# SLebailly/Ignis-MasterThesis

Hardware: AMD Instinct MI355X
Metric: Mrays/s (primary+secondary) at fixed spp; per-pixel L2 vs CPU ref (higher is better)
Workload: dtype f32; 1 GPU; diamond_scene.json 1000x1000, 256 spp = 32 iterations x spi 8, path tracer max_depth 64, seed 0; scene=diamond_scene.json, width=1000, height=1000, spp=256, spi=8, parallelism=single GPU

## Files before the change

ignis-masterthesis_amd/csrc/igx_device.hip:

```cpp
#include "igx.h"

#include "device_math.h"
#include "device_scene.h"
#include "igx_kernels.h"
#include "../host/bvh_build.h"
#include "../host/light_select.h"
#include "../host/lds_plan.h"
#include "../host/aov_plan.h"
#include "../host/film_tools.h"

#include <hip/hip_runtime.h>

#include <algorithm>
#include <array>
#include <chrono>
#include <map>
#include <cmath>
#include <cstring>
#include <condition_variable>
#include <deque>
#include <memory>
#include <mutex>
#include <string>
#include <thread>
#include <vector>
#include <type_traits>

using namespace igxd;

#ifndef IGX_PART
#define IGX_PART 0
#endif

namespace igxh {

constexpr int BLOCK = 256;
constexpr int BLOCK_WIDE = LDS_PLAN_BLOCK_WIDE;
static_assert(BLOCK == LDS_PLAN_BLOCK, "host/lds_plan.h plans for BLOCK-thread blocks");
[[maybe_unused]] constexpr int MAX_BLOCKS_PER_CU = 8;
[[maybe_unused]] constexpr int MAX_STACK = 128;
constexpr int MAX_BOUNCES = 256;
constexpr long long MAX_CHUNK_PATHS = 1ll << 27;
constexpr int SLOT_BITS = 27;
constexpr uint32_t SLOT_MASK = (1u << SLOT_BITS) - 1;
[[maybe_unused]] constexpr int MAX_ENCLOSING = 31;
static_assert(MAX_CHUNK_PATHS <= (1ll << SLOT_BITS), "path slots must fit the slot bits");
#ifndef EXTEND_WAVES
#define EXTEND_WAVES 4
#endif
#ifndef EXTEND_WAVES_FULL
#define EXTEND_WAVES_FULL 3
#endif
#ifndef EXTEND_WAVES_LDS
#define EXTEND_WAVES_LDS 4
#endif


constexpr int NSH = 64;
constexpr int CSTRIDE = 16;
constexpr int CROW = NSH * CSTRIDE;
// ... 589 lines not shown
            if (st.cls)
                for (int k = 0; k < 16; ++k)
                    if (st.cls[20 + k]) atomicAdd(&stats[54 + k], st.cls[20 + k]);
        }
    }
}

template <class CountOf>
__device__ __forceinline__ int take_group(int* work, int& s, uint64_t& done, int n, CountOf count_of, int claimed = -1) {
    unsigned long long* const done_mask = reinterpret_cast<unsigned long long*>(work + CROW);
    for (;;) {
        if (!((done >> s) & 1ull)) {
            int v = claimed;
            claimed = -1;
            if (v < 0) {
                v = 0;
                if (lane_id() == 0) v = atomicAdd(work + s * CSTRIDE, 1);
                v = __builtin_amdgcn_readfirstlane(v);
            }
            if (v * 64 < n) return v;
            if (lane_id() == 0 && !((__hip_atomic_load(done_mask, __ATOMIC_RELAXED, __HIP_MEMORY_SCOPE_AGENT) >> s) & 1ull))
                atomicOr(done_mask, 1ull << s);
            done |= 1ull << s;
        }
        unsigned long long m = 0;
        if (lane_id() == 0) m = __hip_atomic_load(done_mask, __ATOMIC_RELAXED, __HIP_MEMORY_SCOPE_AGENT);
        done |= (uint64_t)(uint32_t)__builtin_amdgcn_readfirstlane((int)(uint32_t)m) |
                ((uint64_t)(uint32_t)__builtin_amdgcn_readfirstlane((int)(uint32_t)(m >> 32)) << 32);
        const uint64_t open = ~done;
        if (!open) return -1;
        const int r = (s + 1) & (NSH - 1);
        const uint64_t rot = (open >> r) | (r ? (open << (NSH - r)) : 0ull);
        s = (r + __ffsll((unsigned long long)rot) - 1) & (NSH - 1);
        n = count_of(s);
    }
}

__device__ __forceinline__ PathState camera_path(const FrameArgs& fa, const SceneView& sv, int i) {
    const GenPath g = gen_path(fa, sv, i);
    PathState ps;
    ps.o = g.o;
    ps.d = g.d;
    ps.counter = g.counter;
    ps.seed = g.seed;
    ps.depth = g.depth;
    ps.slot = i;
    ps.contrib = mk(1, 1, 1);
    ps.inv_pdf = 0;
    ps.eta = 1.0f;
    ps.inside = -1;
    return ps;
}

template <int V0, bool STATS, bool LDS, int BT = BLOCK>
__global__ void __launch_bounds__(BT, LDS ? EXTEND_WAVES_LDS : (variant_full(V0) ? EXTEND_WAVES_FULL : EXTEND_WAVES)) k_extend(FrameArgs fa, SceneView gsv, PathBuf in, PathBuf out, ShadowBuf sh,
                                                  float4* L, KernelCounters kc, int tail_threshold) {
    static_assert(BT == BLOCK || (LDS && BT == BLOCK_WIDE), "the wide block is the LDS-staged kernel's");
    constexpr bool SHADE_LDS = BT > BLOCK;
    constexpr int V = LDS ? kernel_variant(V0, true) : (EXTEND_TREELET ? kernel_variant(V0, false) : V0);
    __shared__ int stack_mem[LDS_STACK * BT];
    extern __shared__ float4 lds_scene[];
    const TStack ts = make_tstack<BT>(stack_mem, LDS_STACK, gsv.spill);
    const bool gen = fa.gen_n > 0;
    if (!gen && row_total(kc.cnt_in) <= tail_threshold) return;
    const SceneView sv = LDS ? stage_scene_lds<BT, SHADE_LDS>(gsv, lds_scene) : stage_treelet<BT>(gsv, lds_scene);
    TraceStats st{0, 0, 0, 0, 0, 0, 0};
    __shared__ unsigned long long cls_mem[STATS ? BT / 64 * 36 : 1];
    if constexpr (STATS) {
        st.cls = cls_mem + 36 * (threadIdx.x >> 6);
        if (lane_id() < 36) st.cls[lane_id()] = 0;
    }
    const WaveWork w = wave_work<BT>();
    int s = w.s;
    auto count_of = [&](int sh_) {
        if (gen) {
            const int g = gen_shard_count(fa.gen_n, sh_);
            return ShardCount{g, g, g};
        }
        return shard_count(kc.cnt_in, sh_);
    };
    ShardCount sc = count_of(s);
    uint64_t done = 0;
    int p0 = w.k * 64;
    int claimed = -1;
    unsigned long long t_last = STATS ? __builtin_amdgcn_s_memtime() : 0;
    for (;;) {
        if (fa.dynamic) {
            const int g = take_group(kc.work, s, done, sc.n, [&](int sh_) {
                sc = count_of(sh_);
                return sc.n;
            }, claimed);
            if (g < 0) break;
            p0 = g * 64;
        } else if (p0 >= sc.n) {
            break;
        }
        if (STATS) phase_mark(st, t_last, 3);
        const int ns = sc.n;
        int* const c_out = kc.cnt_out + s * CSTRIDE;
        int* const c_sh = kc.cnt_shadow + s * CSTRIDE;
        const int q = p0 + lane_id();
        const int pos = (fa.reverse && !gen) ? ns - 1 - q : q;
        bool alive = false, has_shadow = false, has_l = false;
        PathState ps;
        ShadowRec sr;
        f3 Lacc = mk(0, 0, 0);
        ps.depth = 0;
        if (q < ns) {
            if (gen) {
                const int i = ((pos >> 6) << 12) | (s << 6) | (pos & 63);
                ps = camera_path(fa, sv, i);
                if (variant_full(V0) && IGX_AOV && fa.aov_di) fa.aov_di[i] = fa.aov_nee[i] = make_float4(0, 0, 0, 0);
            } else {
                ps = load_path(in, path_index(in, s, pos, sc));
            }
            if (!STATS && ps.depth > 0) alive = extend_step<STATS, V>(fa, sv, ts, ps, Lacc, has_l, has_shadow, sr, st);
// ... 794 lines not shown
[[maybe_unused]] constexpr size_t TREELET_FRONT = 1280;

inline long long row_total(const Slot& s, int row) {
    if (row == 0) return s.n0;
    long long t = 0;
    const int* r = s.pinned + (size_t)row * CROW;
    for (int k = 0; k < NSH; ++k) t += r[k * CSTRIDE] + r[k * CSTRIDE + 1] + r[k * CSTRIDE + 2];
    return t;
}

}

using namespace igxh;

struct igx_device {
    int hip_device = 0;
    hipStream_t stream = nullptr;
    hipStream_t stream2 = nullptr;
    hipStream_t tail_stream = nullptr;
    std::string last_error;
    int num_cus = 256;
    size_t mem_total = 0;
    bool timing = false;
    bool instrument = false;
    int64_t capacity_opt = 0;
    int64_t slot_budget_mb = 0;
    int stream_slots = 2;
    int concurrent_opt = 1;
    int concurrent_start_pct = 10;
    int tail_pairs_opt = -1;
    int64_t treelet_opt = -1;
    bool tree_dirty = true;
    int tree_ext = 0, tree_shadow = 0;
    int64_t tail_opt = -1;
    int64_t tail_last_opt = -1;
    bool fuse_generate = true;
    int split_opt = -1;
    int refill_opt = -1;
    int shadow_ifif_opt = -1;
    int64_t lds_scene_max = 48 * 1024;
    size_t lds_scene_bytes = 0;
    int lds_shading_opt = -1;
    int64_t lds_shading_max = 48 * 1024;
    size_t lds_shading_bytes = 0;
    int ext_block = BLOCK;
    size_t lds_shading_tab[LDS_TAB_COUNT] = {};
    size_t lds_per_block = 64 * 1024;
    size_t table_bytes = 0;
    size_t shading_bytes = 0;
    int leaf_size = 4;
    int classify_opt = 4;
    int shadow_classes_opt = 1;
    int shadow_optimistic_opt = -1;
    int dynamic_opt = DYN_EXTEND | DYN_REFILL_TRACE | DYN_REFILL_SHADOW;
    int group_order_opt = -1;
    int face_normals_opt = 1;
    int face_shade_opt = 1;
    float sah_node_cost = 1.0f;
    int bvh_bins = 32;
    int bvh_bins_tlas = 32;
    bool spatial_splits = false;
    bool rebuild_bvh = false;
    bool has_scene = false;
    std::vector<void*> scene_allocs;
    SceneView sv{};
    igx_camera cam_desc{};
    int variant = 0;
    int bvh_width = 2;
    bool quantized = false;
    int quantize_opt = -1;
    int nf4 = 4;
    int bvh_width_opt = 0;
    bool full_shading = false;
    bool full_shading_opt = false;
    bool enclosing_opt = true;
    int scene_depth = 0;
    int* spill_main = nullptr;
    int* spill_tail = nullptr;
    int* spill_shadow = nullptr;
    int* spill_main2 = nullptr;
    hipStream_t shadow_stream = nullptr;
    int overlap_shadow_opt = 1;
    Slot slots[2];
    int next_slot = 0;
    unsigned long long* dstats = nullptr;
    unsigned long long* tail_counts = nullptr;
    float* ray_list = nullptr;
    size_t ray_list_cap = 0;
    float* fb = nullptr;
    size_t fb_count = 0;
    bool aov_on = false;
    float* aov_fb[2] = {nullptr, nullptr};
    int fb_w = 0, fb_h = 0;
    uint64_t iteration_count = 0;
    int info_mode = INFO_OFF;
    bool info_follow_specular = false;
    int info_max_depth = 8;
    float* info_fb[AOV_INFO_COUNT] = {nullptr, nullptr, nullptr};
    uint64_t info_count[AOV_INFO_COUNT] = {0, 0, 0};
    std::vector<std::pair<hipEvent_t, hipEvent_t>> info_timed;
    void* post_buf[4] = {nullptr, nullptr, nullptr, nullptr};
    size_t post_cap[4] = {0, 0, 0, 0};
    igx_stats stats{};
    int async_opt = 1;
    struct AsyncRender* async = nullptr;
    int host_wait_us = 20;
// ... 18 lines not shown
#define HIPCHK(expr)                                                                                  \
    do {                                                                                              \
        hipError_t e_ = (expr);                                                                       \
        if (e_ != hipSuccess)                                                                         \
            return fail(dev, e_ == hipErrorOutOfMemory ? IGX_ERR_OUT_OF_MEMORY : IGX_ERR_HIP,         \
                        std::string(#expr) + ": " + hipGetErrorString(e_));                           \
    } while (0)

template <typename T>
igx_status upload(igx_device* dev, const std::vector<T>& v, const T** out) {
    size_t bytes = std::max<size_t>(v.size() * sizeof(T), 16);
    void* p = nullptr;
    HIPCHK(hipMalloc(&p, bytes));
    dev->scene_allocs.push_back(p);
    if (!v.empty()) HIPCHK(hipMemcpy(p, v.data(), v.size() * sizeof(T), hipMemcpyHostToDevice));
    *out = reinterpret_cast<const T*>(p);
    return IGX_OK;
}

void free_scene(igx_device* dev) {
    for (void* p : dev->scene_allocs) (void)hipFree(p);
    dev->scene_allocs.clear();
    dev->spill_main = dev->spill_tail = dev->spill_shadow = dev->spill_main2 = nullptr;
    dev->has_scene = false;
}

int max_grid(const igx_device* dev) {
    return std::max(GRID_QUANTUM, dev->num_cus * MAX_BLOCKS_PER_CU / GRID_QUANTUM * GRID_QUANTUM);
}

igx_status configure_stack(igx_device* dev) {
    const int need = dev->scene_depth;
    const int extra = std::max(0, need - LDS_STACK);
    dev->variant = (dev->bvh_width >= 4 ? 2 : 0) | (extra > 0 ? 1 : 0) | (dev->full_shading ? 4 : 0) | (dev->quantized ? VARIANT_Q4 : 0);
    const size_t threads = (size_t)max_grid(dev) * BLOCK;
    for (int k = 0; k < 4; ++k) {
        int*& old = k == 0 ? dev->spill_main : k == 1 ? dev->spill_tail : k == 2 ? dev->spill_shadow : dev->spill_main2;
        if (old) {
            auto it = std::find(dev->scene_allocs.begin(), dev->scene_allocs.end(), (void*)old);
            if (it != dev->scene_allocs.end()) dev->scene_allocs.erase(it);
            (void)hipFree(old);
            old = nullptr;
        }
        void* p = nullptr;
        HIPCHK(hipMalloc(&p, std::max<size_t>(16, (size_t)extra * threads * sizeof(int))));
        dev->scene_allocs.push_back(p);
        (k == 0 ? dev->spill_main : k == 1 ? dev->spill_tail : k == 2 ? dev->spill_shadow : dev->spill_main2) = static_cast<int*>(p);
    }
    dev->sv.spill = dev->spill_main;
    return IGX_OK;
}

void free_slot_buffers(Slot& s) {
    void* ptrs[] = {s.pa.p0, s.pa.p1, s.pa.p2, s.pa.p3, s.pb.p0, s.pb.p1, s.pb.p2, s.pb.p3, s.sh.s0, s.sh.s1, s.sh.s2, s.L, s.hb.h, s.hb.prim,
                    s.aov_di, s.aov_nee};
    for (void* p : ptrs)
        if (p) (void)hipFree(p);
    s.pa = PathBuf{};
    s.pb = PathBuf{};
    s.sh = ShadowBuf{};
    s.hb = HitBuf{};
    s.L = nullptr;
    s.aov_di = s.aov_nee = nullptr;
    s.cap = 0;
    s.shard_cap = 0;
}

igx_status ensure_slot(igx_device* dev, Slot& s, size_t cap, bool hits, bool region_c, bool aov) {
    if (!s.ctr) {
        HIPCHK(hipMalloc((void**)&s.ctr, CTR_INTS * sizeof(int)));
        HIPCHK(hipHostMalloc((void**)&s.pinned, CTR_INTS * sizeof(int), hipHostMallocDefault));
        HIPCHK(hipEventCreateWithFlags(&s.done, hipEventDisableTiming));
        std::memset(s.pinned, 0, CTR_INTS * sizeof(int));
    }
    if (s.cap >= cap && (!hits || s.hb.h) && (!region_c || s.pa.c_base) && (!aov || s.aov_di)) return IGX_OK;
    free_slot_buffers(s);
    const int shard_cap = (int)((cap + 64 * NSH - 1) / (64 * NSH)) * 64;
    const size_t recs = (size_t)shard_cap * NSH;
    auto alloc4 = [&](float4** p, size_t k) -> igx_status { HIPCHK(hipMalloc((void**)p, k * sizeof(float4))); return IGX_OK; };
    igx_status st;
    const size_t precs = region_c ? 2 * recs : recs;
    if ((st = alloc4(&s.pa.p0, precs)) || (st = alloc4(&s.pa.p1, precs)) || (st = alloc4(&s.pa.p2, precs))) return st;
    HIPCHK(hipMalloc((void**)&s.pa.p3, precs * sizeof(float2)));
    if ((st = alloc4(&s.pb.p0, precs)) || (st = alloc4(&s.pb.p1, precs)) || (st = alloc4(&s.pb.p2, precs))) return st;
    HIPCHK(hipMalloc((void**)&s.pb.p3, precs * sizeof(float2)));
    s.pa.c_base = s.pb.c_base = region_c ? (int)recs : 0;
    if ((st = alloc4(&s.sh.s0, recs)) || (st = alloc4(&s.sh.s1, recs)) || (st = alloc4(&s.sh.s2, recs))) return st;
    if ((st = alloc4(&s.L, cap))) return st;
    if (aov && ((st = alloc4(&s.aov_di, cap)) || (st = alloc4(&s.aov_nee, cap)))) return st;
    if (hits) {
        if ((st = alloc4(&s.hb.h, recs))) return st;
        HIPCHK(hipMalloc((void**)&s.hb.prim, recs * sizeof(int)));
    }
    s.pa.shard_cap = s.pb.shard_cap = s.sh.shard_cap = shard_cap;
    s.cap = cap;
    s.shard_cap = shard_cap;
    return IGX_OK;
}

hipEvent_t slot_event(Slot& s) {
    if (s.ev_next >= s.ev_pool.size()) {
        hipEvent_t e;
        (void)hipEventCreate(&e);
        s.ev_pool.push_back(e);
    }
    return s.ev_pool[s.ev_next++];
}

int grid_for(igx_device* dev, long long items, int blocks_per_cu, int block = BLOCK) {
    const long long q = NSH / (block / 64);
    long long need = (items + block - 1) / block;
    long long cap = (long long)dev->num_cus * std::min(blocks_per_cu, MAX_BLOCKS_PER_CU * BLOCK / block);
    long long g = std::min((need + q - 1) / q * q, std::max(q, cap / q * q));
    return (int)std::max(q, g);
}

#endif

constexpr size_t SPLIT_TABLE_BYTES = 64u << 20;
#ifndef GROUP_ORDER_AUTO
#define GROUP_ORDER_AUTO 0
#endif
inline bool use_tail_pairs(const igx_device* dev) {
    return dev->lds_scene_bytes == 0 && (dev->tail_pairs_opt < 0 ? true : dev->tail_pairs_opt != 0);
}
inline size_t tree_bytes(const igx_device* dev, int nodes) { return (size_t)nodes * dev->nf4 * 16; }
inline int refill_min(const igx_device* dev) { return dev->refill_opt >= 0 ? dev->refill_opt : 16; }
inline bool use_refill(const igx_device* dev) {
    return refill_min(dev) > 0 && (dev->lds_scene_bytes == 0 || dev->refill_opt > 0);
}
inline bool use_split(const igx_device* dev) {
    return dev->split_opt >= 0 ? dev->split_opt != 0 : (dev->lds_scene_bytes == 0 && dev->table_bytes > SPLIT_TABLE_BYTES);
}
inline bool use_shadow_ifif(const igx_device* dev) {
    return dev->shadow_ifif_opt >= 0 ? dev->shadow_ifif_opt != 0 : use_split(dev);
}
inline bool use_shadow_optimistic(const igx_device* dev, bool split, bool aovs) {
    if (dev->shadow_optimistic_opt == 0 || split || aovs) return false;
    return dev->shadow_optimistic_opt > 0 || (dev->shadow_classes_opt && dev->sv.num_enc > 0);
}
// ... 5 lines not shown
        case 1: MACRO(1); break;              \
        case 2: MACRO(2); break;              \
        case 3: MACRO(3); break;              \
        case 2 | VARIANT_Q4: MACRO(130); break; \
        default: MACRO(131); break;           \
        }                                     \
    } while (0)
#define IGX_DISPATCH_VARIANT8(v, MACRO)       \
    do {                                      \
        switch ((v) & (7 | VARIANT_Q4)) {     \
        case 0: MACRO(0); break;              \
        case 1: MACRO(1); break;              \
        case 2: MACRO(2); break;              \
        case 3: MACRO(3); break;              \
        case 4: MACRO(4); break;              \
        case 5: MACRO(5); break;              \
        case 6: MACRO(6); break;              \
        case 7: MACRO(7); break;              \
        case 2 | VARIANT_Q4: MACRO(130); break; \
        case 3 | VARIANT_Q4: MACRO(131); break; \
        case 6 | VARIANT_Q4: MACRO(134); break; \
        default: MACRO(135); break;           \
        }                                     \
    } while (0)

template <bool STATS>
void launch_extend_wide(igx_device* dev, Slot& s, int grid, const FrameArgs& fa, const PathBuf& in, const PathBuf& out,
                        const KernelCounters& kc, int tail) {
    const size_t dyn = lds_pad16(dev->lds_scene_bytes) + dev->lds_shading_bytes;
#define L_EXTW(S) hipLaunchKernelGGL((k_extend<S, STATS, true, BLOCK_WIDE>), dim3(grid), dim3(BLOCK_WIDE), dyn, dev->stream, fa, dev->sv, in, out, s.sh, s.L, kc, tail)
    IGX_DISPATCH_VARIANT8(dev->variant, L_EXTW);
#undef L_EXTW
}
template <typename K>
hipError_t raise_dynamic_lds(K kernel, size_t dyn) {
    static std::map<std::pair<const void*, int>, size_t> raised;
    int d = 0;
    (void)hipGetDevice(&d);
    const void* const fn = reinterpret_cast<const void*>(kernel);
    size_t& have = raised[{fn, d}];
    if (dyn <= have) return hipSuccess;
    const hipError_t e = hipFuncSetAttribute(fn, hipFuncAttributeMaxDynamicSharedMemorySize, (int)dyn);
    if (e == hipSuccess) have = dyn;
    return e;
}
template <bool STATS>
hipError_t extend_wide_prepare(int v, size_t dyn) {
#define L_PREP(S) return raise_dynamic_lds(k_extend<S, STATS, true, BLOCK_WIDE>, dyn)
    IGX_DISPATCH_VARIANT8(v, L_PREP);
#undef L_PREP
    return hipSuccess;
}

template <bool STATS>
void launch_extend(igx_device* dev, Slot& s, int grid, const FrameArgs& fa, const PathBuf& in, const PathBuf& out,
                   const KernelCounters& kc, int tail) {
    if (dev->ext_block == BLOCK_WIDE) {
        launch_extend_wide<STATS>(dev, s, grid, fa, in, out, kc, tail);
        return;
    }
    if (dev->lds_scene_bytes) {
#define L_EXTL(S) hipLaunchKernelGGL((k_extend<S, STATS, true>), dim3(grid), dim3(BLOCK), dev->lds_scene_bytes, dev->stream, fa, dev->sv, in, out, s.sh, s.L, kc, tail)
        IGX_DISPATCH_VARIANT8(dev->variant, L_EXTL);
#undef L_EXTL
        return;
    }
    SceneView tsv = dev->sv;
    tsv.tree_n = dev->tree_ext;
#define L_EXT(S) hipLaunchKernelGGL((k_extend<S, STATS, false>), dim3(grid), dim3(BLOCK), tree_bytes(dev, tsv.tree_n), dev->stream, fa, tsv, in, out, s.sh, s.L, kc, tail)
    IGX_DISPATCH_VARIANT8(dev->variant, L_EXT);
#undef L_EXT
}
template <bool STATS>
void launch_trace(igx_device* dev, Slot& s, int grid, const FrameArgs& fa, const PathBuf& in, const int* cnt, int tail,
                  int* work) {
    if (use_refill(dev)) {
#define L_TRR(S)                                                                                                        \
    if (dev->lds_scene_bytes)                                                                                            \
        hipLaunchKernelGGL((k_trace_refill<S, STATS, true>), dim3(grid), dim3(BLOCK), dev->lds_scene_bytes, dev->stream, fa, \
                           dev->sv, in, s.hb, cnt, tail, dev->dstats, refill_min(dev), work);                            \
    else                                                                                                                 \
        hipLaunchKernelGGL((k_trace_refill<S, STATS, false>), dim3(grid), dim3(BLOCK), 0, dev->stream, fa, dev->sv, in, s.hb, \
                           cnt, tail, dev->dstats, refill_min(dev), work)
        IGX_DISPATCH_VARIANT(dev->variant, L_TRR);
#undef L_TRR
        return;
    }
    if (dev->lds_scene_bytes) {
#define L_TRL(S) hipLaunchKernelGGL((k_trace<S, STATS, 1, true>), dim3(grid), dim3(BLOCK), dev->lds_scene_bytes, dev->stream, fa, dev->sv, in, s.hb, cnt, tail, dev->dstats)
        IGX_DISPATCH_VARIANT(dev->variant, L_TRL);
#undef L_TRL
        return;
    }
#define L_TR(S) hipLaunchKernelGGL((k_trace<S, STATS, 5, false>), dim3(grid), dim3(BLOCK), 0, dev->stream, fa, dev->sv, in, s.hb, cnt, tail, dev->dstats)
    IGX_DISPATCH_VARIANT(dev->variant, L_TR);
#undef L_TR
}
template <bool STATS>
void launch_shadow(igx_device* dev, Slot& s, int grid, const int* cnt, int* work, hipStream_t strm) {
    SceneView tsv = dev->sv;
    tsv.tree_n = dev->tree_shadow;
    if (strm != dev->stream) tsv.spill = dev->spill_shadow;
    if (use_refill(dev)) {
#define L_SHR(S)                                                                                                        \
    if (dev->lds_scene_bytes)                                                                                            \
        hipLaunchKernelGGL((k_shadow_refill<S, STATS, true>), dim3(grid), dim3(BLOCK), dev->lds_scene_bytes, strm,   \
                           tsv, s.sh, s.L, cnt, dev->dstats, refill_min(dev), work);                                 \
    else                                                                                                                 \
        hipLaunchKernelGGL((k_shadow_refill<S, STATS, false>), dim3(grid), dim3(BLOCK), tree_bytes(dev, tsv.tree_n), strm, \
// ... 233 lines not shown
    s.timed.clear();
    s.ev_next = 0;
    s.pending = false;
    return IGX_OK;
}

igx_status drain(igx_device* dev) {
    igx_status st;
    if ((st = ::wait_idle(dev)) || (st = harvest(dev, dev->slots[0])) || (st = harvest(dev, dev->slots[1]))) return st;
    HIPCHK(hipStreamSynchronize(dev->stream));
    HIPCHK(hipStreamSynchronize(dev->stream2));
    HIPCHK(hipStreamSynchronize(dev->shadow_stream));
    HIPCHK(hipStreamSynchronize(dev->tail_stream));
    for (auto& t : dev->info_timed) {
        float ms = 0;
        if (hipEventElapsedTime(&ms, t.first, t.second) == hipSuccess) dev->stats.ms_generate += ms;
        (void)hipEventDestroy(t.first);
        (void)hipEventDestroy(t.second);
    }
    dev->info_timed.clear();
    unsigned long long tc[2] = {0, 0};
    HIPCHK(hipMemcpy(tc, dev->tail_counts, sizeof(tc), hipMemcpyDeviceToHost));
    HIPCHK(hipMemset(dev->tail_counts, 0, sizeof(tc)));
    dev->stats.bounce_rays += tc[0];
    dev->stats.shadow_rays += tc[1];
    dev->stats.tail_bounce_rays += tc[0];
    dev->stats.tail_shadow_rays += tc[1];
    return IGX_OK;
}

#ifndef LDS_SHADING_AUTO
#define LDS_SHADING_AUTO 1
#endif
constexpr size_t EXTEND_FIXED_LDS = 2 * MAX_ENC_BOXES * sizeof(float4) + BLOCK_WIDE / 64 * 36 * sizeof(unsigned long long);
void configure_lds(igx_device* dev) {
    dev->lds_scene_bytes = dev->lds_shading_bytes = 0;
    dev->ext_block = BLOCK;
    if (!dev->has_scene) return;
    LdsPlanInput in;
    in.traversal_bytes = dev->table_bytes;
    in.traversal_max = dev->lds_scene_max;
    for (int k = 0; k < LDS_TAB_COUNT; ++k) in.shading_bytes[k] = dev->lds_shading_tab[k];
    in.shading_max = dev->lds_shading_max;
    in.shading_on = dev->lds_shading_opt < 0 ? LDS_SHADING_AUTO != 0 : dev->lds_shading_opt != 0;
    in.stack_bytes_per_thread = LDS_STACK * sizeof(int);
    in.fixed_bytes = EXTEND_FIXED_LDS;
    in.lds_per_block = dev->lds_per_block;
    LdsPlan p = plan_lds(in);
    if (p.block_threads == BLOCK_WIDE) {
        const size_t dyn = lds_pad16(p.traversal_bytes) + p.shading_bytes;
        (void)hipSetDevice(dev->hip_device);
        hipError_t e = extend_wide_prepare<false>(dev->variant, dyn);
        if (e == hipSuccess) e = extend_wide_prepare<true>(dev->variant, dyn);
        if (e != hipSuccess) {
            (void)hipGetLastError();
            dev->last_error = std::string("lds_shading: the wide k_extend's LDS block was refused (") + hipGetErrorString(e) +
                              "); keeping the 256-thread layout";
            p.block_threads = BLOCK;
            p.shading_bytes = 0;
        }
    }
    dev->lds_scene_bytes = p.traversal_bytes;
    dev->lds_shading_bytes = p.shading_bytes;
    dev->ext_block = p.block_threads;
}

void configure_treelet(igx_device* dev) {
    dev->tree_ext = dev->tree_shadow = 0;
    dev->tree_dirty = false;
    if (!dev->has_scene || dev->lds_scene_bytes || dev->treelet_opt == 0) return;
    int cap = (int)std::min<size_t>(TREELET_FRONT, (size_t)dev->sv.num_nodes);
    if (dev->treelet_opt > 0) cap = (int)std::min<int64_t>(cap, dev->treelet_opt);
    const int v = dev->variant;
    const bool refill = use_refill(dev);
    auto fit = [&](auto blocks) {
        const int nb0 = blocks((size_t)0);
        int lo = 0, hi = cap;
        while (lo < hi) {
            const int mid = (lo + hi + 1) / 2;
            if (blocks(tree_bytes(dev, mid)) >= nb0) lo = mid;
            else hi = mid - 1;
        }
        return lo;
    };
    if (EXTEND_TREELET) dev->tree_ext = fit([&](size_t t) { return extend_blocks_per_cu<false>(v, 0, t); });
    if (SHADOW_TREELET && !(refill && use_shadow_ifif(dev))) dev->tree_shadow = fit([&](size_t t) { return shadow_blocks_per_cu<false>(v, 0, refill, t); });
}

long long valid_pixels_in_chunk(const FrameArgs& fa) {
    if (fa.num_rays > 0 || fa.tile_size <= 0) return fa.chunk_pixels;
    long long v = 0;
    const long long T = fa.tile_size, TT = T * T;
    const long long c0 = fa.chunk_pixel0, c1 = c0 + fa.chunk_pixels;
    for (long long k = c0 / TT; k * TT < c1; ++k) {
        const long long t = fa.tile_offset + k * fa.tile_stride;
        const long long ty = t / fa.tiles_x, tx = t - ty * fa.tiles_x;
        const long long w = std::max(0ll, std::min(T, fa.width - tx * T)), h = std::max(0ll, std::min(T, fa.height - ty * T));
        auto valid_first = [&](long long m) {
            if (IGX_PIXEL_BLOCKS && (T & 3) == 0) {
                const long long pairs = m / (2 * T), q = m - pairs * 2 * T, nb = q / 8, rem = q - nb * 8;
                const long long y0 = 2 * pairs, c0 = 4 * nb + std::min(rem, 4ll), c1 = 4 * nb + std::max(0ll, rem - 4);
                return std::min(y0, h) * w + (y0 < h ? std::min(c0, w) : 0) + (y0 + 1 < h ? std::min(c1, w) : 0);
            }
            const long long rows = m / T;
            return std::min(rows, h) * w + (rows < h ? std::min(m % T, w) : 0);
        };
// ... 132 lines not shown
        dev->quantize_opt = (int)value;
    }
    else if (k == "tail_pairs") {
        if (value < -1 || value > 1) return fail(dev, IGX_ERR_INVALID_ARGUMENT, "tail_pairs must be -1 (auto), 0 or 1");
        dev->tail_pairs_opt = (int)value;
    }
    else if (k == "stream_slots") {
        if (value != 1 && value != 2) return fail(dev, IGX_ERR_INVALID_ARGUMENT, "stream_slots must be 1 or 2");
        if (value == 1 && dev->slots[1].cap) {
            igx_status st = harvest(dev, dev->slots[1]);
            if (st != IGX_OK) return st;
            free_slot_buffers(dev->slots[1]);
        }
        dev->stream_slots = (int)value;
    }
    else if (k == "slot_budget_mb") {
        if (value < 0) return fail(dev, IGX_ERR_INVALID_ARGUMENT, "slot_budget_mb must be >= 0 (0 = auto)");
        dev->slot_budget_mb = value;
    }
    else if (k == "concurrent_chunks") dev->concurrent_opt = value != 0 ? 1 : 0;
    else if (k == "async_render") dev->async_opt = value != 0 ? 1 : 0;
    else if (k == "denoise_aovs") {
        if (value < INFO_OFF || value > INFO_EVERY)
            return fail(dev, IGX_ERR_INVALID_ARGUMENT, "denoise_aovs must be 0 (off), 1 (first iteration) or 2 (every iteration)");
        dev->info_mode = (int)value;
    }
    else if (k == "denoise_follow_specular") dev->info_follow_specular = value != 0;
    else if (k == "denoise_max_depth") {
        if (value < 0) return fail(dev, IGX_ERR_INVALID_ARGUMENT, "denoise_max_depth must be >= 0");
        dev->info_max_depth = (int)std::min<int64_t>(value, 1 << 20);
    }
    else if (k == "probe_sample") dev->probe_sample_opt = std::max<int64_t>(0, value);
    else if (k == "fail_chunk") dev->fail_chunk_opt = std::max<int64_t>(0, value);
    else if (k == "face_shade") dev->face_shade_opt = value != 0 ? 1 : 0;
    else if (k == "host_wait_us") dev->host_wait_us = (int)std::max<int64_t>(0, std::min<int64_t>(value, 10000));
    else if (k == "concurrent_start_pct") {
        if (value < 0 || value > 100) return fail(dev, IGX_ERR_INVALID_ARGUMENT, "concurrent_start_pct must be 0..100");
        dev->concurrent_start_pct = (int)value;
    }
    else if (k == "tail_threshold") dev->tail_opt = value;
    else if (k == "tail_threshold_last") dev->tail_last_opt = value;
    else if (k == "fuse_generate") dev->fuse_generate = value != 0;
    else if (k == "split") {
        if (value < -1 || value > 1) return fail(dev, IGX_ERR_INVALID_ARGUMENT, "split must be -1 (auto), 0 or 1");
        dev->split_opt = (int)value;
    }
    else if (k == "shadow_ifif") {
        if (value < -1 || value > 1) return fail(dev, IGX_ERR_INVALID_ARGUMENT, "shadow_ifif must be -1 (auto), 0 or 1");
        dev->shadow_ifif_opt = (int)value;
    }
    else if (k == "shadow_optimistic") {
        if (value < -1 || value > 1) return fail(dev, IGX_ERR_INVALID_ARGUMENT, "shadow_optimistic must be -1 (auto), 0 or 1");
        dev->shadow_optimistic_opt = (int)value;
    }
    else if (k == "refill") {
        if (value < -1 || value > 64) return fail(dev, IGX_ERR_INVALID_ARGUMENT, "refill must be -1 (auto) or in [0, 64]");
        dev->refill_opt = (int)value;
    }
    else if (k == "lds_scene_max") {
        dev->lds_scene_max = value;
        configure_lds(dev);
    }
    else if (k == "lds_shading") {
        if (value < -1 || value > 1) return fail(dev, IGX_ERR_INVALID_ARGUMENT, "lds_shading must be -1 (auto), 0 or 1");
        dev->lds_shading_opt = (int)value;
        configure_lds(dev);
    }
    else if (k == "lds_shading_max") {
        dev->lds_shading_max = value;
        configure_lds(dev);
    }
    else if (k == "full_shading") dev->full_shading_opt = value != 0;
    else if (k == "enclosing") dev->enclosing_opt = value != 0;
    else if (k == "bvh_width") {
        if (value != 0 && value != 2 && value != 4) return fail(dev, IGX_ERR_INVALID_ARGUMENT, "bvh_width must be 0 (auto), 2 or 4");
        dev->bvh_width_opt = (int)value;
    }
    else if (k == "spatial_splits") dev->spatial_splits = value != 0;
    else if (k == "rebuild_bvh") dev->rebuild_bvh = value != 0;
    else if (k == "dynamic") dev->dynamic_opt = (int)(value & 15);
    else if (k == "group_order") {
        if (value < -1 || value > 1) return fail(dev, IGX_ERR_INVALID_ARGUMENT, "group_order must be -1 (auto), 0 (A, B, C) or 1 (C, B, A)");
        dev->group_order_opt = (int)value;
    }
    else if (k == "face_normals") dev->face_normals_opt = value != 0;
    else if (k == "bvh_bins") {
        if (value < 2 || value > 4096) return fail(dev, IGX_ERR_INVALID_ARGUMENT, "bvh_bins must be in [2, 4096]");
        dev->bvh_bins = (int)value;
    }
    else if (k == "bvh_bins_tlas") {
        if (value < 2 || value > 4096) return fail(dev, IGX_ERR_INVALID_ARGUMENT, "bvh_bins_tlas must be in [2, 4096]");
        dev->bvh_bins_tlas = (int)value;
    }
    else if (k == "path_classes") {
        if (value < 0 || value > 4) return fail(dev, IGX_ERR_INVALID_ARGUMENT, "path_classes must be in [0, 4]");
        dev->classify_opt = (int)value;
    }
    else if (k == "sah_node_cost_pct") {
        if (value < 10 || value > 2000) return fail(dev, IGX_ERR_INVALID_ARGUMENT, "sah_node_cost_pct must be in [10, 2000]");
        dev->sah_node_cost = (float)value / 100.0f;
    }
    else if (k == "bvh_leaf_size") {
        if (value < 1 || value > 16) return fail(dev, IGX_ERR_INVALID_ARGUMENT, "bvh_leaf_size must be in [1, 16]");
        dev->leaf_size = (int)value;
    } else return fail(dev, IGX_ERR_INVALID_ARGUMENT, "unknown option '" + k + "'");
    return IGX_OK;
// ... 1915 lines not shown
```

ignis-masterthesis_amd/ignis_amd/_native.py:

```python
import ctypes as C
import os

_PKG_DIR = os.path.dirname(os.path.abspath(__file__))
LIB_PATH = os.environ.get("IGX_LIB_PATH") or os.path.join(os.path.dirname(_PKG_DIR), "libigx.so")



class Mesh(C.Structure):
    _fields_ = [("num_vertices", C.c_uint32), ("num_faces", C.c_uint32),
                ("vertices", C.POINTER(C.c_float)), ("normals", C.POINTER(C.c_float)),
                ("texcoords", C.POINTER(C.c_float)), ("indices", C.POINTER(C.c_uint32))]


class Shape(C.Structure):
    _fields_ = [("type", C.c_int32), ("mesh", C.c_int32), ("sphere", C.c_float * 4),
                ("bbox_min", C.c_float * 3), ("bbox_max", C.c_float * 3), ("is_plane", C.c_int32),
                ("plane_origin", C.c_float * 3), ("plane_x", C.c_float * 3), ("plane_y", C.c_float * 3),
                ("plane_tex", C.c_float * 8), ("ref_bvh", C.c_void_p), ("ref_bvh_bytes", C.c_uint64)]


class Entity(C.Structure):
    _fields_ = [("shape", C.c_int32), ("material", C.c_int32), ("flags", C.c_uint32),
                ("to_global", C.c_float * 12), ("to_local", C.c_float * 12), ("normal", C.c_float * 9),
                ("bbox_min", C.c_float * 3), ("bbox_max", C.c_float * 3)]
# ... 49 lines not shown

class DbTable(C.Structure):
    _fields_ = [("data", C.c_void_p), ("bytes", C.c_uint64), ("lookups", C.POINTER(LookupEntry)), ("count", C.c_uint64)]


class DatabaseView(C.Structure):
    _fields_ = [("entities", DbTable), ("shapes", DbTable), ("trimesh_type_id", C.c_uint32),
                ("sphere_type_id", C.c_uint32), ("trimesh_primbvh", DbTable),
                ("scene_bvh_leaves", C.POINTER(DbTable)), ("num_scene_bvhs", C.c_uint32),
                ("scene_bbox_min", C.c_float * 3), ("scene_bbox_max", C.c_float * 3)]


class ShadingView(C.Structure):
    _fields_ = [("film_width", C.c_int32), ("film_height", C.c_int32), ("camera", Camera), ("technique", Technique),
                ("num_materials", C.c_uint32), ("materials", C.POINTER(Material)),
                ("num_lights", C.c_uint32), ("lights", C.POINTER(Light))]



class RenderParams(C.Structure):
    _fields_ = [("width", C.c_int32), ("height", C.c_int32), ("spi", C.c_int32), ("iteration", C.c_int32),
                ("frame", C.c_int32), ("seed", C.c_int32), ("tile_size", C.c_int32), ("tile_offset", C.c_int32),
                ("tile_stride", C.c_int32), ("num_rays", C.c_int32), ("rays", C.POINTER(C.c_float))]


class Stats(C.Structure):
    _fields_ = [("camera_rays", C.c_uint64), ("bounce_rays", C.c_uint64), ("shadow_rays", C.c_uint64),
                ("iterations", C.c_uint64), ("launches_extend", C.c_uint64), ("launches_shadow", C.c_uint64),
                ("ms_extend", C.c_double), ("ms_shadow", C.c_double), ("ms_generate", C.c_double),
                ("ms_resolve", C.c_double), ("ms_render", C.c_double),
                ("node_visits", C.c_uint64), ("leaf_visits", C.c_uint64), ("tri_tests", C.c_uint64),
                ("blas_enters", C.c_uint64), ("shadow_node_visits", C.c_uint64),
                ("shadow_leaf_visits", C.c_uint64), ("shadow_tri_tests", C.c_uint64),
                ("shadow_blas_enters", C.c_uint64), ("shaded_hits", C.c_uint64),
                ("launches_finish", C.c_uint64), ("ms_finish", C.c_double), ("tail_bounce_rays", C.c_uint64),
                ("tail_shadow_rays", C.c_uint64), ("bvh_depth", C.c_int32), ("stack_entries", C.c_int32),
                ("extend_rays", C.c_uint64), ("extend_paths_out", C.c_uint64),
                ("launches_trace", C.c_uint64), ("ms_trace", C.c_double),
                ("wave_node_iters", C.c_uint64), ("wave_leaf_iters", C.c_uint64),
                ("shadow_wave_node_iters", C.c_uint64), ("shadow_wave_leaf_iters", C.c_uint64),
                ("bvh_width", C.c_int32), ("node_bytes", C.c_int32),
                ("lds_scene_bytes", C.c_int32), ("shadow_blocks_per_cu", C.c_int32),
                ("table_bytes", C.c_uint64), ("shading_bytes", C.c_uint64),
                ("extend_cycles_load", C.c_uint64), ("extend_cycles_trace", C.c_uint64),
                ("extend_cycles_shade", C.c_uint64), ("extend_cycles_store", C.c_uint64),
                ("slot_bytes", C.c_uint64), ("treelet_nodes", C.c_int32 * 4),
                ("extend_class_cycles", C.c_uint64 * 8), ("extend_class_groups", C.c_uint64 * 4),
                ("extend_class_node_iters", C.c_uint64 * 4), ("extend_class_node_visits", C.c_uint64 * 4),
                ("shadow_class_groups", C.c_uint64 * 2), ("shadow_class_node_iters", C.c_uint64 * 2),
                ("shadow_class_node_visits", C.c_uint64 * 2), ("shadow_class_cycles", C.c_uint64 * 2),
                ("shadow_class_occluded", C.c_uint64 * 2), ("tlas_node_visits", C.c_uint64),
                ("hot_node_visits", C.c_uint64 * 3), ("extend_class_shade_cycles", C.c_uint64 * 16),
                ("shadow_class_rays", C.c_uint64 * 2),
                ("lds_shading_bytes", C.c_int32), ("extend_block_threads", C.c_int32)]

    def as_dict(self):
        return {name: (list(getattr(self, name)) if isinstance(getattr(self, name), C.Array) else getattr(self, name))
                for name, _ in self._fields_}


class TonemapSettings(C.Structure):
    _fields_ = [("method", C.c_int32), ("use_gamma", C.c_int32), ("scale", C.c_float), ("exposure_factor", C.c_float),
                ("exposure_offset", C.c_float)]


class ImageInfoSettings(C.Structure):
    _fields_ = [("scale", C.c_float), ("bins", C.c_int32),
                ("histogram_r", C.POINTER(C.c_int32)), ("histogram_g", C.POINTER(C.c_int32)),
                ("histogram_b", C.POINTER(C.c_int32)), ("histogram_l", C.POINTER(C.c_int32)),
                ("acquire_error_stats", C.c_int32), ("acquire_histogram", C.c_int32)]


class ImageInfoOutput(C.Structure):
    _fields_ = [("min", C.c_float), ("max", C.c_float), ("avg", C.c_float), ("soft_min", C.c_float),
                ("soft_max", C.c_float), ("median", C.c_float), ("inf_count", C.c_int32), ("nan_count", C.c_int32),
                ("neg_count", C.c_int32)]


EXPORTED_SYMBOLS = [
    "igx_scene_load_file", "igx_scene_load_string", "igx_scene_get_desc", "igx_scene_free", "igx_write_exr",
    "igx_scene_from_database", "igx_scene_find_material", "igx_scene_entity_name",
    "igx_create", "igx_destroy", "igx_last_error", "igx_version", "igx_set_option", "igx_upload_scene",
    "igx_render", "igx_get_framebuffer", "igx_framebuffer_device_ptr", "igx_get_aov", "igx_aov_device_ptr",
    "igx_pack_tiles", "igx_clear", "igx_get_stats", "igx_reset_stats", "igx_trace_hits", "igx_trace_occlusion", "igx_synchronize", "igx_wait_ready",
    "igx_render_iterations", "igx_objscene_create", "igx_objscene_free", "igx_objscene_add",
    "igx_objscene_set_property", "igx_scene_from_objects", "igx_set_camera",
    "igx_clear_aov", "igx_aov_iteration_count", "igx_write_exr_layers",
    "igx_tonemap", "igx_imageinfo", "igx_tonemap_film", "igx_imageinfo_film",
]

_lib = None


def lib():
    global _lib
    if _lib is not None:
        return _lib
    if not os.path.exists(LIB_PATH):
        raise RuntimeError(f"libigx.so not found at {LIB_PATH}; build it with `make -C ignis-masterthesis_amd`")
    L = C.CDLL(LIB_PATH)
    vp = C.c_void_p
    L.igx_scene_load_file.argtypes = [C.c_char_p, C.c_char_p, C.c_size_t]
    L.igx_scene_load_file.restype = vp
    L.igx_scene_load_string.argtypes = [C.c_char_p, C.c_char_p, C.c_char_p, C.c_size_t]
    L.igx_scene_load_string.restype = vp
    L.igx_scene_from_database.argtypes = [C.POINTER(DatabaseView), C.POINTER(ShadingView), C.c_char_p, C.c_size_t]
    L.igx_scene_from_database.restype = vp
# ... 63 lines not shown
```

include/igx.h:

```cpp
#ifndef IGX_H
#define IGX_H

#include <stddef.h>
#include <stdint.h>

#include "igx_scene.h"

#ifdef __cplusplus
extern "C" {
#endif

typedef enum igx_status {
    IGX_OK = 0,
    IGX_ERR_INVALID_ARGUMENT = 1,
    IGX_ERR_HIP = 2,
    IGX_ERR_OUT_OF_MEMORY = 3,
    IGX_ERR_NO_SCENE = 4,
    IGX_ERR_UNSUPPORTED = 5
} igx_status;

typedef struct igx_device igx_device;

typedef struct igx_render_params {
    int32_t width, height;
// ... 4 lines not shown
    int32_t tile_size, tile_offset, tile_stride;
    int32_t num_rays;
    const float* rays;
} igx_render_params;

typedef struct igx_stats {
    uint64_t camera_rays;
    uint64_t bounce_rays;
    uint64_t shadow_rays;
    uint64_t iterations;
    uint64_t launches_extend;
    uint64_t launches_shadow;
    double ms_extend;
    double ms_shadow;
    double ms_generate;
    double ms_resolve;
    double ms_render;
    uint64_t node_visits, leaf_visits, tri_tests, blas_enters;
    uint64_t shadow_node_visits, shadow_leaf_visits, shadow_tri_tests, shadow_blas_enters;
    uint64_t shaded_hits;
    uint64_t launches_finish;
    double ms_finish;
    uint64_t tail_bounce_rays, tail_shadow_rays;
    int32_t bvh_depth;
    int32_t stack_entries;
    uint64_t extend_rays;
    uint64_t extend_paths_out;
    uint64_t launches_trace;
    double ms_trace;
    uint64_t wave_node_iters;
    uint64_t wave_leaf_iters;
    uint64_t shadow_wave_node_iters;
    uint64_t shadow_wave_leaf_iters;
    int32_t bvh_width;
    int32_t node_bytes;
    int32_t lds_scene_bytes;
    int32_t shadow_blocks_per_cu;
    uint64_t table_bytes;
    uint64_t shading_bytes;
    uint64_t extend_cycles_load, extend_cycles_trace, extend_cycles_shade, extend_cycles_store;
    uint64_t slot_bytes;
    int32_t treelet_nodes[4];
    uint64_t extend_class_cycles[8];
    uint64_t extend_class_groups[4];
    uint64_t extend_class_node_iters[4];
    uint64_t extend_class_node_visits[4];
    uint64_t shadow_class_groups[2], shadow_class_node_iters[2], shadow_class_node_visits[2];
    uint64_t shadow_class_cycles[2], shadow_class_occluded[2];
    uint64_t tlas_node_visits, hot_node_visits[3];
    uint64_t extend_class_shade_cycles[16];
    uint64_t shadow_class_rays[2];
    int32_t lds_shading_bytes;
    int32_t extend_block_threads;
} igx_stats;

igx_status igx_create(int hip_device, igx_device** out);
igx_status igx_destroy(igx_device* dev);
const char* igx_last_error(const igx_device* dev);
const char* igx_version(void);

igx_status igx_set_option(igx_device* dev, const char* key, int64_t value);

igx_status igx_upload_scene(igx_device* dev, const igx_scene_desc* desc);

igx_status igx_set_camera(igx_device* dev, const igx_camera* camera);

igx_status igx_render(igx_device* dev, const igx_render_params* params);
igx_status igx_render_iterations(igx_device* dev, const igx_render_params* params, int32_t count);
igx_status igx_synchronize(igx_device* dev);
igx_status igx_wait_ready(igx_device* dev);

igx_status igx_get_framebuffer(igx_device* dev, float* host_rgb, size_t count, uint64_t* iteration_count);
igx_status igx_framebuffer_device_ptr(igx_device* dev, float** dev_ptr, size_t* count);
igx_status igx_get_aov(igx_device* dev, const char* name, float* host_rgb, size_t count, uint64_t* iteration_count);
igx_status igx_aov_device_ptr(igx_device* dev, const char* name, float** dev_ptr, size_t* count);
igx_status igx_aov_iteration_count(igx_device* dev, const char* name, uint64_t* iteration_count);
igx_status igx_pack_tiles(igx_device* dev, const igx_render_params* params, float* dst_device, size_t count);
igx_status igx_clear(igx_device* dev);
igx_status igx_clear_aov(igx_device* dev, const char* name);

typedef struct {
    int32_t method;
    int32_t use_gamma;
    float scale;
    float exposure_factor, exposure_offset;
} igx_tonemap_settings;
typedef struct {
    float scale;
    int32_t bins;
    int32_t *histogram_r, *histogram_g, *histogram_b, *histogram_l;
    int32_t acquire_error_stats;
    int32_t acquire_histogram;
} igx_imageinfo_settings;
typedef struct {
    float min, max, avg;
    float soft_min, soft_max, median;
    int32_t inf_count, nan_count, neg_count;
} igx_imageinfo_output;
igx_status igx_tonemap(igx_device* dev, const char* aov, const igx_tonemap_settings* settings, uint32_t* out_host,
                       size_t pixel_count);
igx_status igx_imageinfo(igx_device* dev, const char* aov, const igx_imageinfo_settings* settings, igx_imageinfo_output* out);
igx_status igx_tonemap_film(igx_device* dev, const float* film_dev, int32_t width, int32_t height,
                            const igx_tonemap_settings* settings, uint32_t* out_pixels, int32_t out_on_device);
igx_status igx_imageinfo_film(igx_device* dev, const float* film_dev, int32_t width, int32_t height,
                              const igx_imageinfo_settings* settings, igx_imageinfo_output* out);

// ... 13 lines not shown
```

Measured before the change: 14780 Mrays/s.

## Add specialized generate/bounce k_extend shapes with constant-folded frame args

Adds a SHAPE template parameter to k_extend. For the common configuration (dynamic, classify 4, one shadow class, no ray input, no MIS AOVs), the kernel hard-codes those frame-argument fields and derives the stream pointers, shadow pointers and counter rows from a single base pointer. Path and shadow buffers are now allocated as one contiguous block each so those derived offsets are valid. A host check picks the generate or bounce variant when the buffers are packed, and falls back to the generic kernel otherwise. The aim is to let the compiler drop dead branches and save registers or scalar loads, at the cost of more kernel instantiations and a tighter coupling between allocation layout and kernel assumptions.

```diff
diff --git a/ignis-masterthesis_amd/csrc/igx_device.hip b/ignis-masterthesis_amd/csrc/igx_device.hip
--- a/ignis-masterthesis_amd/csrc/igx_device.hip
+++ b/ignis-masterthesis_amd/csrc/igx_device.hip
@@ -6,6 +6,7 @@
 #include "../host/bvh_build.h"
 #include "../host/light_select.h"
 #include "../host/lds_plan.h"
+#include "../host/extend_shape.h"
 #include "../host/aov_plan.h"
 #include "../host/film_tools.h"
 
@@ -701,16 +702,44 @@
     return ps;
 }
 
-template <int V0, bool STATS, bool LDS, int BT = BLOCK>
-__global__ void __launch_bounds__(BT, LDS ? EXTEND_WAVES_LDS : (variant_full(V0) ? EXTEND_WAVES_FULL : EXTEND_WAVES)) k_extend(FrameArgs fa, SceneView gsv, PathBuf in, PathBuf out, ShadowBuf sh,
+template <int V0, bool STATS, bool LDS, int BT = BLOCK, int SHAPE = EXTEND_GENERIC>
+__global__ void __launch_bounds__(BT, LDS ? EXTEND_WAVES_LDS : (variant_full(V0) ? EXTEND_WAVES_FULL : EXTEND_WAVES)) k_extend(FrameArgs fa_arg, SceneView gsv, PathBuf in, PathBuf out, ShadowBuf sh,
                                                   float4* L, KernelCounters kc, int tail_threshold) {
     static_assert(BT == BLOCK || (LDS && BT == BLOCK_WIDE), "the wide block is the LDS-staged kernel's");
+    static_assert(SHAPE == EXTEND_GENERIC || !STATS, "the instrumented kernel is generic");
+    FrameArgs fa = fa_arg;
+    if constexpr (SHAPE != EXTEND_GENERIC) {
+        fa.dynamic = 1;
+        fa.reverse = 0;
+        fa.classify = EXTEND_SHAPE_CLASSIFY;
+        fa.shadow_classes = 1;
+        fa.num_rays = 0;
+        fa.rays = nullptr;
+        fa.aov_di = fa.aov_nee = nullptr;
+        if constexpr (SHAPE == EXTEND_BOUNCE) fa.gen_n = 0;
+        const int cap = out.shard_cap;
+        const size_t recs = (size_t)NSH * cap;
+        auto derive = [&](PathBuf& b) {
+            b.shard_cap = cap;
+            b.c_base = NSH * cap;
+            b.p1 = b.p0 + 2 * recs;
+            b.p2 = b.p0 + 4 * recs;
+            b.p3 = reinterpret_cast<float2*>(b.p0 + 6 * recs);
+        };
+        derive(out);
+        if constexpr (SHAPE == EXTEND_BOUNCE) derive(in);
+        sh.shard_cap = cap;
+        sh.s1 = sh.s0 + recs;
+        sh.s2 = sh.s0 + 2 * recs;
+        kc.cnt_shadow = kc.cnt_in + CROW;
+        kc.cnt_out = kc.cnt_in + 2 * CROW;
+    }
     constexpr bool SHADE_LDS = BT > BLOCK;
     constexpr int V = LDS ? kernel_variant(V0, true) : (EXTEND_TREELET ? kernel_variant(V0, false) : V0);
     __shared__ int stack_mem[LDS_STACK * BT];
     extern __shared__ float4 lds_scene[];
     const TStack ts = make_tstack<BT>(stack_mem, LDS_STACK, gsv.spill);
-    const bool gen = fa.gen_n > 0;
+    const bool gen = SHAPE == EXTEND_GENERATE ? true : SHAPE == EXTEND_BOUNCE ? false : fa.gen_n > 0;
     if (!gen && row_total(kc.cnt_in) <= tail_threshold) return;
     const SceneView sv = LDS ? stage_scene_lds<BT, SHADE_LDS>(gsv, lds_scene) : stage_treelet<BT>(gsv, lds_scene);
     TraceStats st{0, 0, 0, 0, 0, 0, 0};
@@ -1611,6 +1640,7 @@
     int classify_opt = 4;
     int shadow_classes_opt = 1;
     int shadow_optimistic_opt = -1;
+    int extend_shapes_opt = -1;
     int dynamic_opt = DYN_EXTEND | DYN_REFILL_TRACE | DYN_REFILL_SHADOW;
     int group_order_opt = -1;
     int face_normals_opt = 1;
@@ -1735,8 +1765,7 @@
 }
 
 void free_slot_buffers(Slot& s) {
-    void* ptrs[] = {s.pa.p0, s.pa.p1, s.pa.p2, s.pa.p3, s.pb.p0, s.pb.p1, s.pb.p2, s.pb.p3, s.sh.s0, s.sh.s1, s.sh.s2, s.L, s.hb.h, s.hb.prim,
-                    s.aov_di, s.aov_nee};
+    void* ptrs[] = {s.pa.p0, s.pb.p0, s.sh.s0, s.L, s.hb.h, s.hb.prim, s.aov_di, s.aov_nee};
     for (void* p : ptrs)
         if (p) (void)hipFree(p);
     s.pa = PathBuf{};
@@ -1763,12 +1792,16 @@
     auto alloc4 = [&](float4** p, size_t k) -> igx_status { HIPCHK(hipMalloc((void**)p, k * sizeof(float4))); return IGX_OK; };
     igx_status st;
     const size_t precs = region_c ? 2 * recs : recs;
-    if ((st = alloc4(&s.pa.p0, precs)) || (st = alloc4(&s.pa.p1, precs)) || (st = alloc4(&s.pa.p2, precs))) return st;
-    HIPCHK(hipMalloc((void**)&s.pa.p3, precs * sizeof(float2)));
-    if ((st = alloc4(&s.pb.p0, precs)) || (st = alloc4(&s.pb.p1, precs)) || (st = alloc4(&s.pb.p2, precs))) return st;
-    HIPCHK(hipMalloc((void**)&s.pb.p3, precs * sizeof(float2)));
+    for (PathBuf* b : {&s.pa, &s.pb}) {
+        HIPCHK(hipMalloc((void**)&b->p0, precs * (3 * sizeof(float4) + sizeof(float2))));
+        b->p1 = b->p0 + precs;
+        b->p2 = b->p0 + 2 * precs;
+        b->p3 = reinterpret_cast<float2*>(b->p0 + 3 * precs);
+    }
     s.pa.c_base = s.pb.c_base = region_c ? (int)recs : 0;
-    if ((st = alloc4(&s.sh.s0, recs)) || (st = alloc4(&s.sh.s1, recs)) || (st = alloc4(&s.sh.s2, recs))) return st;
+    if ((st = alloc4(&s.sh.s0, 3 * recs))) return st;
+    s.sh.s1 = s.sh.s0 + recs;
+    s.sh.s2 = s.sh.s0 + 2 * recs;
     if ((st = alloc4(&s.L, cap))) return st;
     if (aov && ((st = alloc4(&s.aov_di, cap)) || (st = alloc4(&s.aov_nee, cap)))) return st;
     if (hits) {
@@ -1880,9 +1913,92 @@
     return hipSuccess;
 }
 
+void launch_extend_shaped_wide(igx_device* dev, Slot& s, int grid, ExtendShape shape, const FrameArgs& fa, const PathBuf& in,
+                               const PathBuf& out, const KernelCounters& kc, int tail);
+hipError_t extend_shaped_wide_prepare(int v, size_t dyn);
+void launch_extend_shaped_lds(igx_device* dev, Slot& s, int grid, ExtendShape shape, const FrameArgs& fa, const PathBuf& in,
+                              const PathBuf& out, const KernelCounters& kc, int tail);
+void launch_extend_shaped_global(igx_device* dev, Slot& s, int grid, ExtendShape shape, const FrameArgs& fa, const PathBuf& in,
+                                 const PathBuf& out, const KernelCounters& kc, int tail);
+#define IGX_SHAPED(S, LDS_, BT_, dyn_, sv_)                                                                                        \
+    if (shape == EXTEND_GENERATE)                                                                                                  \
+        hipLaunchKernelGGL((k_extend<S, false, LDS_, BT_, EXTEND_GENERATE>), dim3(grid), dim3(BT_), dyn_, dev->stream, fa, sv_, in, \
+                           out, s.sh, s.L, kc, tail);                                                                              \
+    else                                                                                                                           \
+        hipLaunchKernelGGL((k_extend<S, false, LDS_, BT_, EXTEND_BOUNCE>), dim3(grid), dim3(BT_), dyn_, dev->stream, fa, sv_, in,   \
+                           out, s.sh, s.L, kc, tail)
+#if IGX_PART == 7
+void launch_extend_shaped_wide(igx_device* dev, Slot& s, int grid, ExtendShape shape, const FrameArgs& fa, const PathBuf& in,
+                               const PathBuf& out, const KernelCounters& kc, int tail) {
+    const size_t dyn = lds_pad16(dev->lds_scene_bytes) + dev->lds_shading_bytes;
+#define L_EXTW(S) IGX_SHAPED(S, true, BLOCK_WIDE, dyn, dev->sv)
+    IGX_DISPATCH_VARIANT8(dev->variant, L_EXTW);
+#undef L_EXTW
+}
+hipError_t extend_shaped_wide_prepare(int v, size_t dyn) {
+#define L_PREP(S)                                                                                           \
+    {                                                                                                       \
+        const hipError_t e = raise_dynamic_lds(k_extend<S, false, true, BLOCK_WIDE, EXTEND_GENERATE>, dyn); \
+        return e != hipSuccess ? e : raise_dynamic_lds(k_extend<S, false, true, BLOCK_WIDE, EXTEND_BOUNCE>, dyn); \
+    }
+    IGX_DISPATCH_VARIANT8(v, L_PREP);
+#undef L_PREP
+    return hipSuccess;
+}
+#endif
+#if IGX_PART == 8
+void launch_extend_shaped_lds(igx_device* dev, Slot& s, int grid, ExtendShape shape, const FrameArgs& fa, const PathBuf& in,
+                              const PathBuf& out, const KernelCounters& kc, int tail) {
+#define L_EXTL(S) IGX_SHAPED(S, true, BLOCK, dev->lds_scene_bytes, dev->sv)
+    IGX_DISPATCH_VARIANT8(dev->variant, L_EXTL);
+#undef L_EXTL
+}
+#endif
+#if IGX_PART == 9
+void launch_extend_shaped_global(igx_device* dev, Slot& s, int grid, ExtendShape shape, const FrameArgs& fa, const PathBuf& in,
+                                 const PathBuf& out, const KernelCounters& kc, int tail) {
+    SceneView tsv = dev->sv;
+    tsv.tree_n = dev->tree_ext;
+#define L_EXT(S) IGX_SHAPED(S, false, BLOCK, tree_bytes(dev, tsv.tree_n), tsv)
+    IGX_DISPATCH_VARIANT8(dev->variant, L_EXT);
+#undef L_EXT
+}
+#endif
+#undef IGX_SHAPED
+
+inline ExtendShape launch_shape(const igx_device* dev, bool instrumented, const FrameArgs& fa, const PathBuf& pin, const PathBuf& out,
+                                const ShadowBuf& sh, const KernelCounters& kc) {
+    ExtendShapeInput in;
+    in.extend_shapes = dev->extend_shapes_opt;
+    in.instrument = instrumented;
+    in.gen_n = fa.gen_n;
+    in.dynamic = fa.dynamic;
+    in.reverse = fa.reverse;
+    in.classify = fa.classify;
+    in.shadow_classes = fa.shadow_classes;
+    in.num_rays = fa.num_rays;
+    in.mis_aovs = fa.aov_di != nullptr || fa.aov_nee != nullptr;
+    const auto packed = [&](const PathBuf& b) {
+        const size_t recs = (size_t)NSH * b.shard_cap;
+        return b.shard_cap == out.shard_cap && b.c_base == NSH * b.shard_cap && b.p1 == b.p0 + 2 * recs && b.p2 == b.p0 + 4 * recs &&
+               b.p3 == reinterpret_cast<const float2*>(b.p0 + 6 * recs);
+    };
+    const size_t srecs = (size_t)NSH * sh.shard_cap;
+    in.streams_packed = packed(pin) && packed(out) && sh.shard_cap == out.shard_cap && sh.s1 == sh.s0 + srecs && sh.s2 == sh.s0 + 2 * srecs &&
+                        kc.cnt_shadow == kc.cnt_in + CROW && kc.cnt_out == kc.cnt_in + 2 * CROW;
+    return pick_extend_shape(in);
+}
+
 template <bool STATS>
 void launch_extend(igx_device* dev, Slot& s, int grid, const FrameArgs& fa, const PathBuf& in, const PathBuf& out,
                    const KernelCounters& kc, int tail) {
+    if (const ExtendShape shape = launch_shape(dev, STATS, fa, in, out, s.sh, kc); shape != EXTEND_GENERIC) {
+        ++dev->stats.launches_extend_shaped[shape == EXTEND_GENERATE ? 0 : 1];
+        if (dev->ext_block == BLOCK_WIDE) launch_extend_shaped_wide(dev, s, grid, shape, fa, in, out, kc, tail);
+        else if (dev->lds_scene_bytes) launch_extend_shaped_lds(dev, s, grid, shape, fa, in, out, kc, tail);
+        else launch_extend_shaped_global(dev, s, grid, shape, fa, in, out, kc, tail);
+        return;
+    }
     if (dev->ext_block == BLOCK_WIDE) {
         launch_extend_wide<STATS>(dev, s, grid, fa, in, out, kc, tail);
         return;
@@ -2222,6 +2338,7 @@
         (void)hipSetDevice(dev->hip_device);
         hipError_t e = extend_wide_prepare<false>(dev->variant, dyn);
         if (e == hipSuccess) e = extend_wide_prepare<true>(dev->variant, dyn);
+        if (e == hipSuccess) e = extend_shaped_wide_prepare(dev->variant, dyn);
         if (e != hipSuccess) {
             (void)hipGetLastError();
             dev->last_error = std::string("lds_shading: the wide k_extend's LDS block was refused (") + hipGetErrorString(e) +
@@ -2460,6 +2577,10 @@
     else if (k == "shadow_optimistic") {
         if (value < -1 || value > 1) return fail(dev, IGX_ERR_INVALID_ARGUMENT, "shadow_optimistic must be -1 (auto), 0 or 1");
         dev->shadow_optimistic_opt = (int)value;
+    }
+    else if (k == "extend_shapes") {
+        if (value < -1 || value > 1) return fail(dev, IGX_ERR_INVALID_ARGUMENT, "extend_shapes must be -1 (auto), 0 or 1");
+        dev->extend_shapes_opt = (int)value;
     }
     else if (k == "refill") {
         if (value < -1 || value > 64) return fail(dev, IGX_ERR_INVALID_ARGUMENT, "refill must be -1 (auto) or in [0, 64]");
diff --git a/ignis-masterthesis_amd/host/extend_shape.h b/ignis-masterthesis_amd/host/extend_shape.h
--- /dev/null
+++ b/ignis-masterthesis_amd/host/extend_shape.h
@@ -0,0 +1,34 @@
+#pragma once
+
+namespace igxh {
+
+enum ExtendShape { EXTEND_GENERIC = 0, EXTEND_GENERATE = 1, EXTEND_BOUNCE = 2 };
+
+constexpr int EXTEND_SHAPE_CLASSIFY = 4;
+
+struct ExtendShapeInput {
+    int extend_shapes = -1;
+    bool instrument = false;
+    int gen_n = 0;
+    int dynamic = 0;
+    int reverse = 0;
+    int classify = 0;
+    int shadow_classes = 0;
+    int num_rays = 0;
+    bool mis_aovs = false;
+    bool streams_packed = true;
+};
+
+#ifndef EXTEND_SHAPES_AUTO
+#define EXTEND_SHAPES_AUTO 1
+#endif
+
+inline ExtendShape pick_extend_shape(const ExtendShapeInput& in) {
+    const int opt = in.extend_shapes < 0 ? EXTEND_SHAPES_AUTO : in.extend_shapes;
+    if (opt == 0 || in.instrument) return EXTEND_GENERIC;
+    if (!in.dynamic || in.reverse || in.classify != EXTEND_SHAPE_CLASSIFY || in.shadow_classes != 1 || in.num_rays > 0 || in.mis_aovs || !in.streams_packed)
+        return EXTEND_GENERIC;
+    return in.gen_n > 0 ? EXTEND_GENERATE : EXTEND_BOUNCE;
+}
+
+}
diff --git a/ignis-masterthesis_amd/ignis_amd/_native.py b/ignis-masterthesis_amd/ignis_amd/_native.py
--- a/ignis-masterthesis_amd/ignis_amd/_native.py
+++ b/ignis-masterthesis_amd/ignis_amd/_native.py
@@ -125,7 +125,8 @@
                 ("shadow_class_occluded", C.c_uint64 * 2), ("tlas_node_visits", C.c_uint64),
                 ("hot_node_visits", C.c_uint64 * 3), ("extend_class_shade_cycles", C.c_uint64 * 16),
                 ("shadow_class_rays", C.c_uint64 * 2),
-                ("lds_shading_bytes", C.c_int32), ("extend_block_threads", C.c_int32)]
+                ("lds_shading_bytes", C.c_int32), ("extend_block_threads", C.c_int32),
+                ("launches_extend_shaped", C.c_uint64 * 2)]
 
     def as_dict(self):
         return {name: (list(getattr(self, name)) if isinstance(getattr(self, name), C.Array) else getattr(self, name))
diff --git a/include/igx.h b/include/igx.h
--- a/include/igx.h
+++ b/include/igx.h
@@ -80,6 +80,7 @@
     uint64_t shadow_class_rays[2];
     int32_t lds_shading_bytes;
     int32_t extend_block_threads;
+    uint64_t launches_extend_shaped[2];
 } igx_stats;
 
 igx_status igx_create(int hip_device, igx_device** out);
```

Result: faster. 15060 Mrays/s (median of 6 runs) (+1.9%).
